# magenta/ddsp

Hardware: AMD Instinct MI355X
Metric: Msamples/s (Harmonic+FilteredNoise, 16kHz, 100 harmonics) (higher is better)
Workload: dtype f32 (Harmonic wavetables and the FilteredNoise FIR/IR products: 22-bit operands - fp16 hi/lo pairs on the MFMA matrix cores - with fp32 accumulation; everything else plain fp32, the frame phase prefix fp64)

## Files before the change

### ddsp_amd/csrc/filtered_noise_mfma.hip

```cpp
#include <hip/hip_runtime.h>
#include <hip/hip_ext.h>
#include <stdint.h>
#include <cstdlib>
#include <type_traits>
#include "../../include/ddsp_amd.h"
#include "common.h"
#include "split_f16.h"
#include "noise_ir65.h"
#include "profile.h"
#include "filtered_noise_mfma.h"
#include "launch.h"

namespace ddsp {

constexpr int kMfWaves = 8;
constexpr int kMfPW = kMfWaves / 2;
constexpr int kMfRows = 8 * kMfPW;
constexpr int kMfFrames = kMfRows - 2;
constexpr int kMfTile = kMfFrames * 64;
constexpr int kMfTapRowBytes = 17 * 16;
constexpr int kMfTapPlane = kMfRows * kMfTapRowBytes;
constexpr int kMfXStride = 80;
constexpr int kMfXElems = 16 + kMfRows * kMfXStride + 16;
constexpr int kMfXPairs = kMfXElems / 2 + 1;
constexpr int kMfXPlane = kMfWaves == 16 ? 10336 : 5216;
static_assert(kMfXPlane >= kMfXPairs * 4 && kMfXPlane % 16 == 0 && (2 * kMfXPlane / 4) % 32 == 16, "noise plane layout");
constexpr int kMfXOGen = kMfXPlane + 96;
static_assert(kMfXOGen % 16 == 0 && (kMfXOGen / 4) % 32 == 16 && kMfWaves == 8, "noise plane layout, generated noise");
template <bool GEN> struct MfX {
  static constexpr int O = GEN ? kMfXOGen : 2 * kMfXPlane;
  static constexpr int BYTES = GEN ? kMfXOGen + kMfXPlane : 4 * kMfXPlane;
};
struct MfHandoff {
  uint4 frag[kMfPW / 2][4][64];
  float last[kMfRows];
  float tap32[kMfRows];
};

struct MfArgs {
  int N, F, start, scale, fs;
  float inv_fs;
  float bias;
  uint32_t k0, k1;
  uint64_t batch_offset;
  int tiles_per_row, n_tiles;
  FastDiv whole_per_row, fs_div;
  int n_whole;
  const float* x_absmax;
  int bits23;
};

static __constant__ Ir65Frags kIr65Frags = make_ir65_frags();

__device__ __forceinline__ void mf_put4(unsigned char* hrow, int t0, float v0, float v1, float v2, float v3) {
  _Float16 h0, l0, h1, l1, h2, l2, h3, l3;
  split(v0, h0, l0); split(v1, h1, l1); split(v2, h2, l2); split(v3, h3, l3);
  unsigned char* q = hrow + t0 * 2;
  *reinterpret_cast<uint2*>(q) = make_uint2(pack(h0, h1), pack(h2, h3));
  *reinterpret_cast<uint2*>(q + kMfTapPlane) = make_uint2(pack(l0, l1), pack(l2, l3));
}
__device__ __forceinline__ void mf_put4_down(unsigned char* hrow, int t1, bool first, float v0, float v1, float v2, float v3) {
  _Float16 h0, l0, h1, l1, h2, l2, h3, l3;
  split(v0, h0, l0); split(v1, h1, l1); split(v2, h2, l2); split(v3, h3, l3);
  unsigned char* q = hrow + (t1 - 3) * 2;
  *reinterpret_cast<uint16_t*>(q) = __builtin_bit_cast(uint16_t, h3);
  *reinterpret_cast<uint16_t*>(q + kMfTapPlane) = __builtin_bit_cast(uint16_t, l3);
  *reinterpret_cast<uint32_t*>(q + 2) = pack(h2, h1);
  *reinterpret_cast<uint32_t*>(q + kMfTapPlane + 2) = pack(l2, l1);
  if (first) {
    *reinterpret_cast<uint16_t*>(q + 6) = __builtin_bit_cast(uint16_t, h0);
    *reinterpret_cast<uint16_t*>(q + kMfTapPlane + 6) = __builtin_bit_cast(uint16_t, l0);
  }
}

template <bool LO>
__device__ __forceinline__ void mf_put_quad(float4 v, int qd, unsigned char* s_xe, unsigned char* s_xo) {
  _Float16 h0, l0, h1, l1, h2, l2, h3, l3;
  split(v.w, h0, l0);
  split(v.z, h1, l1);
  split(v.y, h2, l2);
  split(v.x, h3, l3);
  const int s = qd >> 4, j = 4 * (qd & 15);
  const int u0 = 16 + kMfXStride * s + 60 - j;
  *reinterpret_cast<uint2*>(s_xe + u0 * 2) = make_uint2(pack(h0, h1), pack(h2, h3));
  if (LO) *reinterpret_cast<uint2*>(s_xe + kMfXPlane + u0 * 2) = make_uint2(pack(l0, l1), pack(l2, l3));
  unsigned char* po = s_xo + (u0 + 1) * 2;
  *reinterpret_cast<uint16_t*>(po) = __builtin_bit_cast(uint16_t, h0);
  *reinterpret_cast<uint32_t*>(po + 2) = pack(h1, h2);
  *reinterpret_cast<uint16_t*>(po + 6) = __builtin_bit_cast(uint16_t, h3);
  if (LO) {
    *reinterpret_cast<uint16_t*>(po + kMfXPlane) = __builtin_bit_cast(uint16_t, l0);
    *reinterpret_cast<uint32_t*>(po + kMfXPlane + 2) = pack(l1, l2);
    *reinterpret_cast<uint16_t*>(po + kMfXPlane + 6) = __builtin_bit_cast(uint16_t, l3);
  }
}

template <bool GEN_NOISE, int NLANES>
__device__ __forceinline__ void mf_noise_tile(int ltid, int b, int z0, const float* __restrict__ x, unsigned char* s_xe,
                                              unsigned char* s_xo, const MfArgs& p) {
  int x_exp = 0;
  if constexpr (!GEN_NOISE) {
    if (p.x_absmax) x_exp = pow2_exponent(p.x_absmax[b]);
  }
  if constexpr (GEN_NOISE) {
    static_assert((8 * kMfRows) % NLANES == 0, "octets per lane");
#pragma unroll
    for (int h = 0; h < 8 * kMfRows / NLANES; ++h) {
      const int oc = ltid + NLANES * h;
      const int i = z0 - 128 + 8 * oc;
      float4 v0 = make_float4(0.f, 0.f, 0.f, 0.f), v1 = v0;
      if (i >= 0 && i < p.N) {
        const U4 r = noise_philox(U4{(uint32_t)(i >> 3), (uint32_t)(p.batch_offset + b), 0u, 0u}, p.k0, p.k1);
        v0 = noise_quad(r, 0);
        v1 = noise_quad(r, 1);
        if (i + 7 >= p.N) {
          if (i + 1 >= p.N) v0.y = 0.f;
          if (i + 2 >= p.N) v0.z = 0.f;
          if (i + 3 >= p.N) v0.w = 0.f;
          if (i + 4 >= p.N) v1.x = 0.f;
          if (i + 5 >= p.N) v1.y = 0.f;
          if (i + 6 >= p.N) v1.z = 0.f;
          v1.w = 0.f;
        }
      }
      mf_put_quad<false>(v0, 2 * oc, s_xe, s_xo);
      mf_put_quad<false>(v1, 2 * oc + 1, s_xe, s_xo);
    }
  } else {
    static_assert((16 * kMfRows) % NLANES == 0, "quads per lane");
#pragma unroll
    for (int h = 0; h < 16 * kMfRows / NLANES; ++h) {
      const int qd = ltid + NLANES * h;
      const int i = z0 - 128 + 4 * qd;
      float4 v = make_float4(0.f, 0.f, 0.f, 0.f);
      if (i >= 0 && i < p.N) {
        if (x == nullptr) {
          v = noise_quad_at((uint32_t)i, p.batch_offset + b, p.k0, p.k1, true);
          if (i + 1 >= p.N) v.y = 0.f;
          if (i + 2 >= p.N) v.z = 0.f;
          if (i + 3 >= p.N) v.w = 0.f;
        } else {
          const float* src = x + (size_t)b * p.N + i;
          if (i + 3 < p.N && ((p.N & 3) == 0)) {
            v = *reinterpret_cast<const float4*>(src);
          } else {
            v.x = src[0];
            if (i + 1 < p.N) v.y = src[1];
            if (i + 2 < p.N) v.z = src[2];
            if (i + 3 < p.N) v.w = src[3];
          }
          if (x_exp) { v.x = ldexpf(v.x, -x_exp); v.y = ldexpf(v.y, -x_exp); v.z = ldexpf(v.z, -x_exp); v.w = ldexpf(v.w, -x_exp); }
        }
      }
      mf_put_quad<true>(v, qd, s_xe, s_xo);
    }
  }
}

template <bool GEN_NOISE, bool FS64>
__global__ __launch_bounds__(64 * kMfWaves, 4) void noise_mfma65_kernel(
    const float* __restrict__ mag , const float* __restrict__ x ,
    float* __restrict__ ctl_out , float* __restrict__ out , MfArgs p) {
  __shared__ __attribute__((aligned(16))) unsigned char s_taps_all[2][2 * kMfTapPlane];
  constexpr int kXO = MfX<GEN_NOISE>::O;
  __shared__ __attribute__((aligned(16))) unsigned char s_x_all[2][MfX<GEN_NOISE>::BYTES];
  __shared__ __attribute__((aligned(16))) std::conditional_t<GEN_NOISE, MfHandoff, uint4> s_hand[2];
  __shared__ __attribute__((aligned(16))) float s_carry[2][kMfPW - 1][128];
  const int tid = threadIdx.x, lane = tid & 63;
  const int wave = __builtin_amdgcn_readfirstlane(tid >> 6);
  const int mi = lane & 15, mg = lane >> 4;
  const int n_my = (p.n_tiles - (int)blockIdx.x + (int)gridDim.x - 1) / (int)gridDim.x;
#define DDSP_MF_TILE(T, b_, z0_, ffirst_, rel0_)                                                        \
  const bool last_ = (T) >= p.n_whole;                                                                  \
  uint32_t tx_;                                                                                         \
  const int bq_ = (int)fastdiv((uint32_t)(T), p.whole_per_row, tx_);                                    \
  const int b_ = last_ ? (T) - p.n_whole : bq_;                                                         \
  const int z0_ = (last_ ? p.tiles_per_row - 1 : (int)tx_) * kMfTile;                                   \
  uint32_t fr_;                                                                                         \
  const int fq_ = (int)fastdiv((uint32_t)(z0_ >= 128 ? z0_ - 128 : 128 - z0_ + p.fs - 1), p.fs_div, fr_); \
  const int ffirst_ = (z0_ >= 128) ? fq_ : -fq_;                                                        \
  const int rel0_ = (z0_ - 128) - ffirst_ * p.fs

  if (wave < kMfPW) {
    constexpr bool HANDOFF = GEN_NOISE;
    const float kLog10 = 2.302585092994046f;
    const bool designer = wave < kMfPW / 2;
    const int rg = wave & (kMfPW / 2 - 1);
    if (designer)
      *reinterpret_cast<uint4*>(s_taps_all[lane >> 5] + (lane & 1) * kMfTapPlane + (16 * rg + ((lane >> 1) & 15)) * kMfTapRowBytes + 256) = make_uint4(0u, 0u, 0u, 0u);
    for (int i = tid; i < 2 * (kMfRows + 1) * 16; i += 64 * kMfPW) {
      unsigned char* const s_xe = s_x_all[i >= (kMfRows + 1) * 16 ? 1 : 0];
      unsigned char* const s_xo = s_xe + kXO;
      const int ii = i >= (kMfRows + 1) * 16 ? i - (kMfRows + 1) * 16 : i;
      const int e = 80 * (ii >> 4) + (ii & 15);
      *reinterpret_cast<uint16_t*>(s_xe + e * 2) = 0;
      *reinterpret_cast<uint16_t*>(s_xo + (e + 1) * 2) = 0;
      if (!GEN_NOISE) {
        *reinterpret_cast<uint16_t*>(s_xe + kMfXPlane + e * 2) = 0;
        *reinterpret_cast<uint16_t*>(s_xo + kMfXPlane + (e + 1) * 2) = 0;
      }
    }
    const int rrow = 16 * rg + mi;
    auto group_unused = [&](int rel0, int z0, int f_first) -> bool {
      if (FS64) return false;
      uint32_t r_;
      const int last_tap_row = (int)fastdiv((uint32_t)(rel0 + 64 * (kMfRows - 1)), p.fs_div, r_);
      const int own_hi = (int)fastdiv((uint32_t)(z0 + kMfTile - 128), p.fs_div, r_) + 2;
      return 16 * rg > last_tap_row && 16 * rg >= own_hi - f_first;
    };
    PackedF4 rq[4];
    float r_last;
    auto fetch_rows = [&](int tick_of_tile) {
      const int T = (int)blockIdx.x + min(max(tick_of_tile, 0), n_my - 1) * (int)gridDim.x;
      DDSP_MF_TILE(T, b, z0, f_first, rel0);
      if (group_unused(rel0, z0, f_first)) return;
      const int rfr = f_first + rrow;
      const float* __restrict__ src = mag + ((size_t)b * p.F + ((rfr >= 0 && rfr < p.F) ? rfr : 0)) * 65;
#pragma unroll
      for (int c4 = 0; c4 < 4; ++c4) rq[c4] = *reinterpret_cast<const PackedF4*>(src + 16 * mg + 4 * c4);
      r_last = src[64];
    };
    auto scale_rows = [&](int T, f16x8& be_hi, f16x8& be_lo, f16x8& bo_hi, f16x8& bo_lo, float& m_last, float& t32) -> bool {
      DDSP_MF_TILE(T, b, z0, f_first, rel0);
      const int own_lo = (z0 == 0) ? 0 : f_first + 2;
      uint32_t own_r;
      const int own_hi = (int)fastdiv((uint32_t)(z0 + kMfTile - 128), p.fs_div, own_r) + 2;
      const int rfr = f_first + rrow;
      const bool rvalid = rfr >= 0 && rfr < p.F;
      if (f_first + 16 * rg > p.F + 1 || group_unused(rel0, z0, f_first)) return false;
      float y[16];
#pragma unroll
      for (int c4 = 0; c4 < 4; ++c4) { y[4 * c4] = rq[c4].x; y[4 * c4 + 1] = rq[c4].y; y[4 * c4 + 2] = rq[c4].z; y[4 * c4 + 3] = rq[c4].w; }
      m_last = r_last;
      if (p.scale & 1) {
#pragma unroll
        for (int c = 0; c < 16; ++c) y[c] = exp_sigmoid_fast(y[c] + p.bias, kLog10, 2.0f, 1e-7f);
        m_last = exp_sigmoid_fast(m_last + p.bias, kLog10, 2.0f, 1e-7f);
      }
      if (!rvalid) {
#pragma unroll
        for (int c = 0; c < 16; ++c) y[c] = 0.0f;
        m_last = 0.0f;
      }
      if (ctl_out && rvalid && rfr >= own_lo && rfr < own_hi) {
        float* __restrict__ dst = ctl_out + ((size_t)b * p.F + rfr) * 65;
#pragma unroll
        for (int c4 = 0; c4 < 4; ++c4)
          *reinterpret_cast<PackedF4*>(dst + 16 * mg + 4 * c4) = PackedF4{y[4 * c4], y[4 * c4 + 1], y[4 * c4 + 2], y[4 * c4 + 3]};
        if (mg == 0) dst[64] = m_last;
      }
      float ve[8], vo[8];
#pragma unroll
      for (int e = 0; e < 8; ++e) { ve[e] = y[2 * e]; vo[e] = y[2 * e + 1]; }
      split8(ve, be_hi, be_lo);
      split8(vo, bo_hi, bo_lo);
      const float* __restrict__ c32 = kIr65.c + 32 * kIrRowStride + 8 * mg;
      float part = (mg == 0) ? m_last * kIr65.c[32 * kIrRowStride + 32] : 0.0f;
#pragma unroll
      for (int e = 0; e < 8; ++e) part = fmaf(c32[e], ve[e], part);
      part += __shfl_xor(part, 16);
      part += __shfl_xor(part, 32);
      t32 = kIr65.win[32] * part;
      return true;
    };
    auto make_noise = [&](int tick) {
      if (tick >= 0 && tick + 1 < n_my) {
        const int T = (int)blockIdx.x + (tick + 1) * (int)gridDim.x;
        DDSP_MF_TILE(T, b, z0, f_first, rel0);
        (void)rel0; (void)f_first;
        unsigned char* const s_xe = s_x_all[(tick + 1) & 1];
        if constexpr (HANDOFF) mf_noise_tile<GEN_NOISE, 64 * kMfPW>(tid, b, z0, x, s_xe, s_xe + kXO, p);
        else mf_noise_tile<GEN_NOISE, 32 * kMfPW>(tid - 32 * kMfPW, b, z0, x, s_xe, s_xe + kXO, p);
      }
    };
    if (!designer) {
      if constexpr (HANDOFF) fetch_rows(1);
#pragma unroll 1
      for (int tick = -1; tick < n_my; ++tick) {
        if constexpr (HANDOFF) {
          if (tick + 2 < n_my) {
            const int T = (int)blockIdx.x + (tick + 2) * (int)gridDim.x;
            MfHandoff& h = s_hand[(tick + 2) & 1];
            f16x8 be_hi, be_lo, bo_hi, bo_lo;
            float m_last, t32;
            if (scale_rows(T, be_hi, be_lo, bo_hi, bo_lo, m_last, t32)) {
              h.frag[rg][0][lane] = __builtin_bit_cast(uint4, be_hi);
              h.frag[rg][1][lane] = __builtin_bit_cast(uint4, be_lo);
              h.frag[rg][2][lane] = __builtin_bit_cast(uint4, bo_hi);
              h.frag[rg][3][lane] = __builtin_bit_cast(uint4, bo_lo);
              if (mg == 0) { h.last[rrow] = m_last; h.tap32[rrow] = t32; }
            }
          }
          fetch_rows(tick + 3);
        }
        make_noise(tick);
        __syncthreads();
      }
    } else {
      f16x8 afr[2][2][2];
#pragma unroll
      for (int mt = 0; mt < 2; ++mt)
#pragma unroll
        for (int par = 0; par < 2; ++par)
#pragma unroll
          for (int hl = 0; hl < 2; ++hl) {
            const uint4 v = *reinterpret_cast<const uint4*>(kIr65Frags.v[mt][par][hl][lane]);
            afr[mt][par][hl] = frag(v.x, v.y, v.z, v.w);
          }
      auto design_rows = [&](unsigned char* s_taps, const f16x8& be_hi, const f16x8& be_lo, const f16x8& bo_hi,
                             const f16x8& bo_lo, float m_last, float t32) {
          unsigned char* __restrict__ hrow = s_taps + rrow * kMfTapRowBytes;
          const f32x4 zero = {0.f, 0.f, 0.f, 0.f};
#pragma unroll
          for (int mt = 0; mt < 2; ++mt) {
            f32x4 ea = __builtin_amdgcn_mfma_f32_16x16x32_f16(afr[mt][0][0], be_hi, zero, 0, 0, 0);
            f32x4 oa = __builtin_amdgcn_mfma_f32_16x16x32_f16(afr[mt][1][0], bo_hi, zero, 0, 0, 0);
            f32x4 ex = __builtin_amdgcn_mfma_f32_16x16x32_f16(afr[mt][0][0], be_lo, zero, 0, 0, 0);
            f32x4 ox = __builtin_amdgcn_mfma_f32_16x16x32_f16(afr[mt][1][0], bo_lo, zero, 0, 0, 0);
            ex = __builtin_amdgcn_mfma_f32_16x16x32_f16(afr[mt][0][1], be_hi, ex, 0, 0, 0);
            ox = __builtin_amdgcn_mfma_f32_16x16x32_f16(afr[mt][1][1], bo_hi, ox, 0, 0, 0);
            const f32x4 ev = combine(ea, ex), ov = combine(oa, ox);
            const int n0 = 16 * mt + 4 * mg;
            float g0[4], g1[4];
#pragma unroll
            for (int r = 0; r < 4; ++r) {
              const int n = n0 + r;
              const float e = fmaf(m_last, kIr65.c[n * kIrRowStride + 32], ev[r]);
              const float o = ov[r];
              g0[r] = kIr65.win[n] * (e + o);
              g1[r] = (n >= 1) ? kIr65.win[64 - n] * (e - o) : 0.0f;
            }
            mf_put4(hrow, 64 + n0, g0[0], g0[1], g0[2], g0[3]);
            mf_put4(hrow, n0, g1[0], g1[1], g1[2], g1[3]);
            mf_put4_down(hrow, 64 - n0, true, g0[0], g0[1], g0[2], g0[3]);
            mf_put4_down(hrow, 128 - n0, n0 != 0, g1[0], g1[1], g1[2], g1[3]);
          }
          if (mg == 0) {
            _Float16 h, l;
            split(t32, h, l);
            const uint16_t hb = __builtin_bit_cast(uint16_t, h), lb = __builtin_bit_cast(uint16_t, l);
            *reinterpret_cast<uint16_t*>(hrow + 96 * 2) = hb;
            *reinterpret_cast<uint16_t*>(hrow + kMfTapPlane + 96 * 2) = lb;
            *reinterpret_cast<uint16_t*>(hrow + 32 * 2) = hb;
            *reinterpret_cast<uint16_t*>(hrow + kMfTapPlane + 32 * 2) = lb;
          }
      };
      fetch_rows(0);
      auto designer_tick = [&](int tick, auto scale_here_tag) {
        constexpr bool SCALE_HERE = decltype(scale_here_tag)::value;
        if (tick + 1 < n_my) {
          const int T = (int)blockIdx.x + (tick + 1) * (int)gridDim.x;
          unsigned char* const s_taps = s_taps_all[(tick + 1) & 1];
          if constexpr (SCALE_HERE) {
            f16x8 be_hi, be_lo, bo_hi, bo_lo;
            float m_last = 0.0f, t32 = 0.0f;
            if (scale_rows(T, be_hi, be_lo, bo_hi, bo_lo, m_last, t32)) design_rows(s_taps, be_hi, be_lo, bo_hi, bo_lo, m_last, t32);
          } else if constexpr (HANDOFF) {
            DDSP_MF_TILE(T, b, z0, f_first, rel0);
            (void)b;
            if (f_first + 16 * rg <= p.F + 1 && !group_unused(rel0, z0, f_first)) {
              const MfHandoff& h = s_hand[(tick + 1) & 1];
              design_rows(s_taps, __builtin_bit_cast(f16x8, h.frag[rg][0][lane]), __builtin_bit_cast(f16x8, h.frag[rg][1][lane]),
                          __builtin_bit_cast(f16x8, h.frag[rg][2][lane]), __builtin_bit_cast(f16x8, h.frag[rg][3][lane]),
                          h.last[rrow], h.tap32[rrow]);
            }
          }
        }
        if (!HANDOFF) fetch_rows(tick + 2);
        if constexpr (HANDOFF) make_noise(tick);
        __syncthreads();
      };
      designer_tick(-1, std::true_type{});
#pragma unroll 1
      for (int tick = 0; tick < n_my; ++tick) designer_tick(tick, std::integral_constant<bool, !HANDOFF>{});
    }
  } else {
    const int cw = wave - kMfPW;
    const int p_first = 4 * cw;
    f32x4 kept = {0.f, 0.f, 0.f, 0.f};
    float* kept_ot = nullptr;
    long kept_n = 0;
    int kept_exp = 0;
    const int xsel = ((mi & 1) ? 0 : kXO) + 2 * kMfXStride * 2 * p_first;
    const int second = mg >> 1;
    const int u4 = 79 + kMfXStride * second - 16 * 4 - mi + 8 * (mg & 1);
    const int a_base0 = xsel + ((u4 + 1) >> 1) * 4;
    const int q0 = mi - 4 * second;
    const int b_off = (q0 >= 0 && q0 <= 7) ? (2 * q0 + (mg & 1)) * 16 : 256;
    const int b_ptr0 = (2 * p_first + second) * kMfTapRowBytes + b_off;
    const int lane_off = 16 * mi + 4 * mg;
    auto flush_kept = [&](int parity) {
      if (cw >= 1 && kept_ot != nullptr && mi < 8) {
        const float4 cr = *reinterpret_cast<const float4*>(&s_carry[parity][cw - 1][lane_off]);
        float v[4] = {kept[0] + cr.x, kept[1] + cr.y, kept[2] + cr.z, kept[3] + cr.w};
        if constexpr (!GEN_NOISE) {
#pragma unroll
          for (int r = 0; r < 4; ++r) v[r] = ldexpf(v[r], kept_exp);
        }
#pragma unroll
        for (int r = 0; r < 4; ++r)
          if (kept_n + lane_off + r >= 0 && kept_n + lane_off + r < p.N) kept_ot[lane_off + r] = v[r];
      }
    };
#pragma unroll 1
    for (int tick = -1; tick < n_my; ++tick) {
      if (tick >= 1) flush_kept((tick - 1) & 1);
      if (tick < 0) {
        const int T = (int)blockIdx.x;
        DDSP_MF_TILE(T, b, z0, f_first, rel0);
        (void)f_first; (void)rel0;
        mf_noise_tile<GEN_NOISE, 64 * kMfPW>(tid - 64 * kMfPW, b, z0, x, s_x_all[0], s_x_all[0] + kXO, p);
      }
      bool active = false;
      if (tick >= 0) {
        const int T = (int)blockIdx.x + tick * (int)gridDim.x;
        DDSP_MF_TILE(T, b, z0, f_first, rel0);
        (void)f_first;
        active = (long)z0 - 128 + 128L * p_first - p.start < (long)p.N;
      }
      if (active) {
        const int T = (int)blockIdx.x + tick * (int)gridDim.x;
        DDSP_MF_TILE(T, b, z0, f_first, rel0);
        (void)f_first;
        const unsigned char* const s_taps = s_taps_all[tick & 1];
        const unsigned char* const s_x = s_x_all[tick & 1];
        float* __restrict__ o = out + (size_t)b * p.N;
        const long n_tile = (long)z0 - 128 + 128L * p_first - p.start;
        const bool interior = n_tile + 128 >= 0 && n_tile + 128 * 4 <= (long)p.N && (((p.start | p.N) & 1) == 0);
        float* __restrict__ ot = o + n_tile;
        int o_exp = 0;
        if constexpr (!GEN_NOISE) {
          if (p.x_absmax) o_exp = pow2_exponent(p.x_absmax[b]);
        }
        f32x4 carry = {0.f, 0.f, 0.f, 0.f};
        int a_hi[2], a_lo[2], b_ptr = b_ptr0;
        DDSP_KEEP_IN_VGPR(b_ptr);
        __builtin_assume((b_ptr & 15) == 0);
#pragma unroll
        for (int k = 0; k < 2; ++k) {
          a_hi[k] = a_base0 + 640 * k; a_lo[k] = a_base0 + 640 * k + kMfXPlane;
          DDSP_KEEP_IN_VGPR(a_hi[k]);
          DDSP_KEEP_IN_VGPR(a_lo[k]);
          __builtin_assume((a_hi[k] & 3) == 0);
          __builtin_assume((a_lo[k] & 3) == 0);
        }
        f16x8 fah[3], fal[3], fbh_in[2], fbl_in[2], fbh, fbl;
        auto load_step = [&](int j, int slot) {
          const int it = j / 5, c = j - 5 * it;
          const PackedU4 qh = *reinterpret_cast<const PackedU4*>(s_x + a_hi[it >> 1] + 32 * (4 - c) + 2 * kMfXStride * 2 * (it & 1));
          fah[slot] = frag(qh.x, qh.y, qh.z, qh.w);
          if constexpr (!GEN_NOISE) {
            const PackedU4 ql = *reinterpret_cast<const PackedU4*>(s_x + a_lo[it >> 1] + 32 * (4 - c) + 2 * kMfXStride * 2 * (it & 1));
            fal[slot] = frag(ql.x, ql.y, ql.z, ql.w);
          }
          if (c == 0) {
            const unsigned char* tr;
            if (FS64) {
              tr = s_taps + b_ptr + 2 * kMfTapRowBytes * it;
            } else {
              const int P = p_first + it;
              const int row = (int)(((float)(rel0 + 128 * P + 64 * second) + 0.5f) * p.inv_fs);
              tr = s_taps + row * kMfTapRowBytes + b_off;
            }
            fbh_in[it & 1] = *reinterpret_cast<const f16x8*>(tr);
            fbl_in[it & 1] = *reinterpret_cast<const f16x8*>(tr + kMfTapPlane);
          }
        };
        auto column_up = [](f16x8 v) {
          typedef int i32x4 __attribute__((ext_vector_type(4)));
          const i32x4 w = __builtin_bit_cast(i32x4, v);
          i32x4 o;
#pragma unroll
          for (int k = 0; k < 4; ++k) {
            const int t = w[k];
            o[k] = __builtin_amdgcn_update_dpp(0, t, 0x111, 0xF, 0xF, true);
          }
          return __builtin_bit_cast(f16x8, o);
        };
        load_step(0, 0);
        load_step(1, 1);
        load_step(2, 2);
        __builtin_amdgcn_sched_barrier(0);
        f32x4 acc = {0.f, 0.f, 0.f, 0.f}, acc_hl = {0.f, 0.f, 0.f, 0.f}, acc_lh = {0.f, 0.f, 0.f, 0.f};
        auto pipeline = [&](auto interior_tag) {
          constexpr bool kInterior = decltype(interior_tag)::value;
#pragma unroll
          for (int j = 0; j < 20; ++j) {
            const int it = j / 5, c = j - 5 * it, slot = j % 3;
            if (c == 0) { fbh = fbh_in[it & 1]; fbl = fbl_in[it & 1]; }
            acc = __builtin_amdgcn_mfma_f32_16x16x32_f16(fah[slot], fbh, acc, 0, 0, 0);
            acc_hl = __builtin_amdgcn_mfma_f32_16x16x32_f16(fah[slot], fbl, acc_hl, 0, 0, 0);
            if constexpr (!GEN_NOISE) acc_lh = __builtin_amdgcn_mfma_f32_16x16x32_f16(fal[slot], fbh, acc_lh, 0, 0, 0);
            __builtin_amdgcn_sched_barrier(0);
            if (j + 3 < 20) load_step(j + 3, slot);
            if (c < 4) { fbh = column_up(fbh); fbl = column_up(fbl); }
            __builtin_amdgcn_sched_barrier(0);
            if (c == 4) {
              const f32x4 comb = combine(acc + carry, acc_hl + acc_lh);
              acc = (f32x4){0.f, 0.f, 0.f, 0.f};
              acc_hl = (f32x4){0.f, 0.f, 0.f, 0.f};
              acc_lh = (f32x4){0.f, 0.f, 0.f, 0.f};
              if (it == 0) {
                kept = comb;
              } else if (mi < 8) {
                const int idx = lane_off + 128 * it;
                f32x4 st4 = comb;
                if constexpr (!GEN_NOISE) {
#pragma unroll
                  for (int r = 0; r < 4; ++r) { const float v = comb[r]; st4[r] = ldexpf(v, o_exp); }
                }
                if (kInterior) {
                  *reinterpret_cast<float2*>(ot + idx) = make_float2(st4[0], st4[1]);
                  *reinterpret_cast<float2*>(ot + idx + 2) = make_float2(st4[2], st4[3]);
                } else {
#pragma unroll
                  for (int r = 0; r < 4; ++r) {
                    const float v = st4[r];
                    if (n_tile + idx + r >= 0 && n_tile + idx + r < p.N) ot[idx + r] = v;
                  }
                }
              }
#pragma unroll
              for (int r = 0; r < 4; ++r) {
                const float v = comb[r];
                carry[r] = __builtin_bit_cast(float, __builtin_amdgcn_update_dpp(0, __builtin_bit_cast(int, v), 0x108, 0xF, 0xF, true));
              }
              if (it == 3 && cw < kMfPW - 1 && mi >= 8)
                *reinterpret_cast<float4*>(&s_carry[tick & 1][cw][lane_off - 128]) = make_float4(comb[0], comb[1], comb[2], comb[3]);
            }
          }
        };
        if (interior) pipeline(std::true_type{});
        else pipeline(std::false_type{});
        kept_ot = ot;
        kept_n = n_tile;
        kept_exp = o_exp;
      } else {
        kept_ot = nullptr;
      }
      __syncthreads();
    }
    flush_kept((n_my - 1) & 1);
  }
#undef DDSP_MF_TILE
}

bool noise_mfma65_ok(int F, int M, int N, int padding, const void* noise, int scale) {
  const int frame_size = (N + F - 1) / F;
  return scale != 0 && M == 65 && padding == 0 && frame_size >= 64 && (frame_size % 64) == 0 && frame_size <= 4096 &&
         (N + frame_size - 1) / frame_size == F && (noise == nullptr || (((uintptr_t)noise) & 15) == 0);
}

__global__ __launch_bounds__(1024) void row_absmax_kernel(const float* __restrict__ x, int N, float* __restrict__ out) {
  __shared__ float s_m[16];
  const float* row = x + (size_t)blockIdx.x * N;
  float m = 0.0f;
  for (int i = threadIdx.x; i < N; i += 1024) m = fmaxf(m, fabsf(row[i]));
  m = wave_max_nonneg_dpp(m);
  if ((threadIdx.x & 63) == 0) s_m[threadIdx.x >> 6] = m;
  __syncthreads();
  if (threadIdx.x == 0) {
    float r = 0.0f;
    for (int w = 0; w < 16; ++w) r = fmaxf(r, s_m[w]);
    out[blockIdx.x] = r;
  }
}

int launch_noise_mfma65(const float* magnitudes, const float* noise, float* audio, float* ctl_magnitudes, int B, int F,
                        int N, int start, float initial_bias, int scale, uint64_t seed, uint64_t batch_offset,
                        int bits23, float* row_scratch , hipStream_t st) {
  MfArgs q;
  q.x_absmax = nullptr; q.bits23 = bits23;
  if (noise) {
    if (!row_scratch) return DDSP_ERR_WORKSPACE;
    hipLaunchKernelGGL(row_absmax_kernel, dim3((unsigned)B), dim3(1024), 0, st, noise, N, row_scratch);
    q.x_absmax = row_scratch;
  }
  const bool lo_planes = noise != nullptr || bits23 != 0;
  q.N = N; q.F = F; q.start = start; q.bias = initial_bias; q.scale = scale;
  q.fs = (N + F - 1) / F; q.inv_fs = 1.0f / (float)q.fs;
  q.k0 = (uint32_t)seed; q.k1 = (uint32_t)(seed >> 32); q.batch_offset = batch_offset;
  q.tiles_per_row = (N + start + kMfTile - 1) / kMfTile;
  q.n_tiles = B * q.tiles_per_row;
  q.whole_per_row = make_fastdiv((uint32_t)(q.tiles_per_row > 1 ? q.tiles_per_row - 1 : 1));
  q.fs_div = make_fastdiv((uint32_t)q.fs);
  q.n_whole = B * (q.tiles_per_row - 1);
  static const int n_cu = [] {
    int dev = 0, v = 0;
    if (hipGetDevice(&dev) != hipSuccess ||
        hipDeviceGetAttribute(&v, hipDeviceAttributeMultiprocessorCount, dev) != hipSuccess || v <= 0)
      v = 256;
    return v;
  }();
  const int slots = n_cu * (kMfWaves == 16 ? 1 : 2);
  const dim3 grid((unsigned)(q.n_tiles < slots ? q.n_tiles : slots));
  hipEvent_t ev0, ev1;
  profile_kernel_events(kNoiseMfma, &ev0, &ev1);
#define DDSP_LAUNCH_MF(GEN, FS64)                                                                                      \
  hipExtLaunchKernelGGL((noise_mfma65_kernel<GEN, FS64>), grid, dim3(64 * kMfWaves), 0, st, ev0, ev1, 0, magnitudes, noise, \
                        ctl_magnitudes, audio, q)
  if (q.fs == 64) { if (lo_planes) DDSP_LAUNCH_MF(false, true); else DDSP_LAUNCH_MF(true, true); }
  else { if (lo_planes) DDSP_LAUNCH_MF(false, false); else DDSP_LAUNCH_MF(true, false); }
#undef DDSP_LAUNCH_MF
  return check_launch();
}

}
```

Measured before the change: 114,600.

## Schedule noise tiles as contiguous per-block runs with carry handoff instead of overlap

Replaces the fixed overlapping tile decomposition (each tile recomputed two frames of halo) with contiguous runs of 128-sample pairs per block, split evenly into tiles. The overlap-add carry is passed between consecutive tiles through shared memory, so halo recomputation is avoided and the work per block is balanced. A rounding-order bitmask reproduces the previous summation order at tile seams. This adds per-tile index math and a cross-tile dependency, and rows with few pairs may underfill tiles.

After: 103,900. -9.3%, worse.

```diff
diff --git a/ddsp_amd/csrc/filtered_noise_mfma.hip b/ddsp_amd/csrc/filtered_noise_mfma.hip
--- a/ddsp_amd/csrc/filtered_noise_mfma.hip
+++ b/ddsp_amd/csrc/filtered_noise_mfma.hip
@@ -16,8 +16,9 @@
 constexpr int kMfWaves = 8;
 constexpr int kMfPW = kMfWaves / 2;
 constexpr int kMfRows = 8 * kMfPW;
-constexpr int kMfFrames = kMfRows - 2;
-constexpr int kMfTile = kMfFrames * 64;
+constexpr int kMfPairs = kMfRows / 2;
+constexpr int kMfRoundGrid = 15;
+constexpr uint32_t kMfRoundLate = 0x888u | (0x888u << kMfRoundGrid);
 constexpr int kMfTapRowBytes = 17 * 16;
 constexpr int kMfTapPlane = kMfRows * kMfTapRowBytes;
 constexpr int kMfXStride = 80;
@@ -43,14 +44,43 @@
   float bias;
   uint32_t k0, k1;
   uint64_t batch_offset;
-  int tiles_per_row, n_tiles;
-  FastDiv whole_per_row, fs_div;
-  int n_whole;
+  FastDiv fs_div;
+  int n_runs, run_q, run_rem, tiles_per_run;
+  FastDiv runs_per_row, tiles_per_run_div;
+  int tile_q[3], tile_rem[3];
   const float* x_absmax;
   int bits23;
 };
 
 static __constant__ Ir65Frags kIr65Frags = make_ir65_frags();
+
+struct MfTileAt {
+  int b;
+  int p0;
+  int np;
+  int f_first;
+  int rel0;
+  bool hist;
+  bool carry_in;
+};
+__device__ __forceinline__ MfTileAt mf_tile_at(const MfArgs& p, int k) {
+  MfTileAt t;
+  uint32_t ti, r;
+  const int ri = (int)fastdiv((uint32_t)k, p.tiles_per_run_div, ti);
+  t.b = (int)fastdiv((uint32_t)((int)blockIdx.x + ri * (int)gridDim.x), p.runs_per_row, r);
+  const int hist_run = r > 0 ? 1 : 0;
+  const int cls = ((int)r < p.run_rem ? 1 : 0) + hist_run;
+  const int tq = cls == 0 ? p.tile_q[0] : cls == 1 ? p.tile_q[1] : p.tile_q[2];
+  const int trem = cls == 0 ? p.tile_rem[0] : cls == 1 ? p.tile_rem[1] : p.tile_rem[2];
+  t.p0 = (int)r * p.run_q + min((int)r, p.run_rem) - hist_run + (int)ti * tq + min((int)ti, trem);
+  t.np = tq + ((int)ti < trem ? 1 : 0);
+  t.hist = hist_run && ti == 0;
+  t.carry_in = ti > 0;
+  uint32_t rel;
+  t.f_first = (int)fastdiv((uint32_t)(128 * t.p0), p.fs_div, rel);
+  t.rel0 = (int)rel;
+  return t;
+}
 
 __device__ __forceinline__ void mf_put4(unsigned char* hrow, int t0, float v0, float v1, float v2, float v3) {
   _Float16 h0, l0, h1, l1, h2, l2, h3, l3;
@@ -96,7 +126,7 @@
 }
 
 template <bool GEN_NOISE, int NLANES>
-__device__ __forceinline__ void mf_noise_tile(int ltid, int b, int z0, const float* __restrict__ x, unsigned char* s_xe,
+__device__ __forceinline__ void mf_noise_tile(int ltid, int b, int zs, const float* __restrict__ x, unsigned char* s_xe,
                                               unsigned char* s_xo, const MfArgs& p) {
   int x_exp = 0;
   if constexpr (!GEN_NOISE) {
@@ -107,9 +137,9 @@
 #pragma unroll
     for (int h = 0; h < 8 * kMfRows / NLANES; ++h) {
       const int oc = ltid + NLANES * h;
-      const int i = z0 - 128 + 8 * oc;
+      const int i = zs + 8 * oc;
       float4 v0 = make_float4(0.f, 0.f, 0.f, 0.f), v1 = v0;
-      if (i >= 0 && i < p.N) {
+      if (i < p.N) {
         const U4 r = noise_philox(U4{(uint32_t)(i >> 3), (uint32_t)(p.batch_offset + b), 0u, 0u}, p.k0, p.k1);
         v0 = noise_quad(r, 0);
         v1 = noise_quad(r, 1);
@@ -131,9 +161,9 @@
 #pragma unroll
     for (int h = 0; h < 16 * kMfRows / NLANES; ++h) {
       const int qd = ltid + NLANES * h;
-      const int i = z0 - 128 + 4 * qd;
+      const int i = zs + 4 * qd;
       float4 v = make_float4(0.f, 0.f, 0.f, 0.f);
-      if (i >= 0 && i < p.N) {
+      if (i < p.N) {
         if (x == nullptr) {
           v = noise_quad_at((uint32_t)i, p.batch_offset + b, p.k0, p.k1, true);
           if (i + 1 >= p.N) v.y = 0.f;
@@ -165,21 +195,11 @@
   constexpr int kXO = MfX<GEN_NOISE>::O;
   __shared__ __attribute__((aligned(16))) unsigned char s_x_all[2][MfX<GEN_NOISE>::BYTES];
   __shared__ __attribute__((aligned(16))) std::conditional_t<GEN_NOISE, MfHandoff, uint4> s_hand[2];
-  __shared__ __attribute__((aligned(16))) float s_carry[2][kMfPW - 1][128];
+  __shared__ __attribute__((aligned(16))) float s_carry[2][kMfPW][128];
   const int tid = threadIdx.x, lane = tid & 63;
   const int wave = __builtin_amdgcn_readfirstlane(tid >> 6);
   const int mi = lane & 15, mg = lane >> 4;
-  const int n_my = (p.n_tiles - (int)blockIdx.x + (int)gridDim.x - 1) / (int)gridDim.x;
-#define DDSP_MF_TILE(T, b_, z0_, ffirst_, rel0_)                                                        \
-  const bool last_ = (T) >= p.n_whole;                                                                  \
-  uint32_t tx_;                                                                                         \
-  const int bq_ = (int)fastdiv((uint32_t)(T), p.whole_per_row, tx_);                                    \
-  const int b_ = last_ ? (T) - p.n_whole : bq_;                                                         \
-  const int z0_ = (last_ ? p.tiles_per_row - 1 : (int)tx_) * kMfTile;                                   \
-  uint32_t fr_;                                                                                         \
-  const int fq_ = (int)fastdiv((uint32_t)(z0_ >= 128 ? z0_ - 128 : 128 - z0_ + p.fs - 1), p.fs_div, fr_); \
-  const int ffirst_ = (z0_ >= 128) ? fq_ : -fq_;                                                        \
-  const int rel0_ = (z0_ - 128) - ffirst_ * p.fs
+  const int n_my = (p.n_runs - (int)blockIdx.x + (int)gridDim.x - 1) / (int)gridDim.x * p.tiles_per_run;
 
   if (wave < kMfPW) {
     constexpr bool HANDOFF = GEN_NOISE;
@@ -201,33 +221,32 @@
       }
     }
     const int rrow = 16 * rg + mi;
-    auto group_unused = [&](int rel0, int z0, int f_first) -> bool {
-      if (FS64) return false;
+    auto group_unused = [&](const MfTileAt& t) -> bool {
       uint32_t r_;
-      const int last_tap_row = (int)fastdiv((uint32_t)(rel0 + 64 * (kMfRows - 1)), p.fs_div, r_);
-      const int own_hi = (int)fastdiv((uint32_t)(z0 + kMfTile - 128), p.fs_div, r_) + 2;
-      return 16 * rg > last_tap_row && 16 * rg >= own_hi - f_first;
+      const int last_tap_row = (int)fastdiv((uint32_t)(t.rel0 + 128 * t.np - 64), p.fs_div, r_);
+      const int own_hi = (int)fastdiv((uint32_t)(t.rel0 + 128 * t.np), p.fs_div, r_);
+      return 16 * rg > last_tap_row && 16 * rg >= own_hi;
     };
     PackedF4 rq[4];
     float r_last;
     auto fetch_rows = [&](int tick_of_tile) {
-      const int T = (int)blockIdx.x + min(max(tick_of_tile, 0), n_my - 1) * (int)gridDim.x;
-      DDSP_MF_TILE(T, b, z0, f_first, rel0);
-      if (group_unused(rel0, z0, f_first)) return;
-      const int rfr = f_first + rrow;
-      const float* __restrict__ src = mag + ((size_t)b * p.F + ((rfr >= 0 && rfr < p.F) ? rfr : 0)) * 65;
+      const MfTileAt t = mf_tile_at(p, min(max(tick_of_tile, 0), n_my - 1));
+      if (group_unused(t)) return;
+      const int rfr = t.f_first + rrow;
+      const float* __restrict__ src = mag + ((size_t)t.b * p.F + ((rfr >= 0 && rfr < p.F) ? rfr : 0)) * 65;
 #pragma unroll
       for (int c4 = 0; c4 < 4; ++c4) rq[c4] = *reinterpret_cast<const PackedF4*>(src + 16 * mg + 4 * c4);
       r_last = src[64];
     };
-    auto scale_rows = [&](int T, f16x8& be_hi, f16x8& be_lo, f16x8& bo_hi, f16x8& bo_lo, float& m_last, float& t32) -> bool {
-      DDSP_MF_TILE(T, b, z0, f_first, rel0);
-      const int own_lo = (z0 == 0) ? 0 : f_first + 2;
+    auto scale_rows = [&](int k, f16x8& be_hi, f16x8& be_lo, f16x8& bo_hi, f16x8& bo_lo, float& m_last, float& t32) -> bool {
+      const MfTileAt t = mf_tile_at(p, k);
+      const int b = t.b, f_first = t.f_first;
       uint32_t own_r;
-      const int own_hi = (int)fastdiv((uint32_t)(z0 + kMfTile - 128), p.fs_div, own_r) + 2;
+      const int own_lo = f_first + (int)fastdiv((uint32_t)(t.rel0 + (t.hist ? 128 : 0)), p.fs_div, own_r);
+      const int own_hi = f_first + (int)fastdiv((uint32_t)(t.rel0 + 128 * t.np), p.fs_div, own_r);
       const int rfr = f_first + rrow;
-      const bool rvalid = rfr >= 0 && rfr < p.F;
-      if (f_first + 16 * rg > p.F + 1 || group_unused(rel0, z0, f_first)) return false;
+      const bool rvalid = rfr < p.F;
+      if (f_first + 16 * rg > p.F + 1 || group_unused(t)) return false;
       float y[16];
 #pragma unroll
       for (int c4 = 0; c4 < 4; ++c4) { y[4 * c4] = rq[c4].x; y[4 * c4 + 1] = rq[c4].y; y[4 * c4 + 2] = rq[c4].z; y[4 * c4 + 3] = rq[c4].w; }
@@ -265,12 +284,10 @@
     };
     auto make_noise = [&](int tick) {
       if (tick >= 0 && tick + 1 < n_my) {
-        const int T = (int)blockIdx.x + (tick + 1) * (int)gridDim.x;
-        DDSP_MF_TILE(T, b, z0, f_first, rel0);
-        (void)rel0; (void)f_first;
+        const MfTileAt t = mf_tile_at(p, tick + 1);
         unsigned char* const s_xe = s_x_all[(tick + 1) & 1];
-        if constexpr (HANDOFF) mf_noise_tile<GEN_NOISE, 64 * kMfPW>(tid, b, z0, x, s_xe, s_xe + kXO, p);
-        else mf_noise_tile<GEN_NOISE, 32 * kMfPW>(tid - 32 * kMfPW, b, z0, x, s_xe, s_xe + kXO, p);
+        if constexpr (HANDOFF) mf_noise_tile<GEN_NOISE, 64 * kMfPW>(tid, t.b, 128 * t.p0, x, s_xe, s_xe + kXO, p);
+        else mf_noise_tile<GEN_NOISE, 32 * kMfPW>(tid - 32 * kMfPW, t.b, 128 * t.p0, x, s_xe, s_xe + kXO, p);
       }
     };
     if (!designer) {
@@ -279,11 +296,10 @@
       for (int tick = -1; tick < n_my; ++tick) {
         if constexpr (HANDOFF) {
           if (tick + 2 < n_my) {
-            const int T = (int)blockIdx.x + (tick + 2) * (int)gridDim.x;
             MfHandoff& h = s_hand[(tick + 2) & 1];
             f16x8 be_hi, be_lo, bo_hi, bo_lo;
             float m_last, t32;
-            if (scale_rows(T, be_hi, be_lo, bo_hi, bo_lo, m_last, t32)) {
+            if (scale_rows(tick + 2, be_hi, be_lo, bo_hi, bo_lo, m_last, t32)) {
               h.frag[rg][0][lane] = __builtin_bit_cast(uint4, be_hi);
               h.frag[rg][1][lane] = __builtin_bit_cast(uint4, be_lo);
               h.frag[rg][2][lane] = __builtin_bit_cast(uint4, bo_hi);
@@ -349,16 +365,14 @@
       auto designer_tick = [&](int tick, auto scale_here_tag) {
         constexpr bool SCALE_HERE = decltype(scale_here_tag)::value;
         if (tick + 1 < n_my) {
-          const int T = (int)blockIdx.x + (tick + 1) * (int)gridDim.x;
           unsigned char* const s_taps = s_taps_all[(tick + 1) & 1];
           if constexpr (SCALE_HERE) {
             f16x8 be_hi, be_lo, bo_hi, bo_lo;
             float m_last = 0.0f, t32 = 0.0f;
-            if (scale_rows(T, be_hi, be_lo, bo_hi, bo_lo, m_last, t32)) design_rows(s_taps, be_hi, be_lo, bo_hi, bo_lo, m_last, t32);
+            if (scale_rows(tick + 1, be_hi, be_lo, bo_hi, bo_lo, m_last, t32)) design_rows(s_taps, be_hi, be_lo, bo_hi, bo_lo, m_last, t32);
           } else if constexpr (HANDOFF) {
-            DDSP_MF_TILE(T, b, z0, f_first, rel0);
-            (void)b;
-            if (f_first + 16 * rg <= p.F + 1 && !group_unused(rel0, z0, f_first)) {
+            const MfTileAt t = mf_tile_at(p, tick + 1);
+            if (t.f_first + 16 * rg <= p.F + 1 && !group_unused(t)) {
               const MfHandoff& h = s_hand[(tick + 1) & 1];
               design_rows(s_taps, __builtin_bit_cast(f16x8, h.frag[rg][0][lane]), __builtin_bit_cast(f16x8, h.frag[rg][1][lane]),
                           __builtin_bit_cast(f16x8, h.frag[rg][2][lane]), __builtin_bit_cast(f16x8, h.frag[rg][3][lane]),
@@ -378,6 +392,7 @@
     const int cw = wave - kMfPW;
     const int p_first = 4 * cw;
     f32x4 kept = {0.f, 0.f, 0.f, 0.f};
+    float kept_late = 0.0f;
     float* kept_ot = nullptr;
     long kept_n = 0;
     int kept_exp = 0;
@@ -390,9 +405,22 @@
     const int b_ptr0 = (2 * p_first + second) * kMfTapRowBytes + b_off;
     const int lane_off = 16 * mi + 4 * mg;
     auto flush_kept = [&](int parity) {
-      if (cw >= 1 && kept_ot != nullptr && mi < 8) {
+      if (cw < 1 || kept_ot == nullptr) return;
+      float cross[4];
+#pragma unroll
+      for (int r = 0; r < 4; ++r) {
+        const float kv = kept[r];
+        cross[r] = __builtin_bit_cast(float, __builtin_amdgcn_update_dpp(0, __builtin_bit_cast(int, kv), 0x108, 0xF, 0xF, true));
+      }
+      if (mi < 8) {
         const float4 cr = *reinterpret_cast<const float4*>(&s_carry[parity][cw - 1][lane_off]);
-        float v[4] = {kept[0] + cr.x, kept[1] + cr.y, kept[2] + cr.z, kept[3] + cr.w};
+        const float crv[4] = {cr.x, cr.y, cr.z, cr.w};
+        float v[4];
+#pragma unroll
+        for (int r = 0; r < 4; ++r) {
+          const float kv = kept[r];
+          v[r] = combine(kv + crv[r] * (1.0f - kept_late), cross[r]) + crv[r] * kept_late;
+        }
         if constexpr (!GEN_NOISE) {
 #pragma unroll
           for (int r = 0; r < 4; ++r) v[r] = ldexpf(v[r], kept_exp);
@@ -406,33 +434,30 @@
     for (int tick = -1; tick < n_my; ++tick) {
       if (tick >= 1) flush_kept((tick - 1) & 1);
       if (tick < 0) {
-        const int T = (int)blockIdx.x;
-        DDSP_MF_TILE(T, b, z0, f_first, rel0);
-        (void)f_first; (void)rel0;
-        mf_noise_tile<GEN_NOISE, 64 * kMfPW>(tid - 64 * kMfPW, b, z0, x, s_x_all[0], s_x_all[0] + kXO, p);
-      }
-      bool active = false;
-      if (tick >= 0) {
-        const int T = (int)blockIdx.x + tick * (int)gridDim.x;
-        DDSP_MF_TILE(T, b, z0, f_first, rel0);
-        (void)f_first;
-        active = (long)z0 - 128 + 128L * p_first - p.start < (long)p.N;
-      }
+        const MfTileAt t0 = mf_tile_at(p, 0);
+        mf_noise_tile<GEN_NOISE, 64 * kMfPW>(tid - 64 * kMfPW, t0.b, 128 * t0.p0, x, s_x_all[0], s_x_all[0] + kXO, p);
+      }
+      const MfTileAt t = mf_tile_at(p, max(tick, 0));
+      const bool active = tick >= 0 && p_first < t.np && 128L * (t.p0 + p_first) - p.start < (long)p.N;
       if (active) {
-        const int T = (int)blockIdx.x + tick * (int)gridDim.x;
-        DDSP_MF_TILE(T, b, z0, f_first, rel0);
-        (void)f_first;
+        const int b = t.b, rel0 = t.rel0;
+        const int n_pairs = t.np - p_first;
+        const bool st_first = cw == 0 && !t.hist;
+        const uint32_t late = kMfRoundLate >> ((uint32_t)(t.p0 + p_first) % (uint32_t)kMfRoundGrid);
         const unsigned char* const s_taps = s_taps_all[tick & 1];
         const unsigned char* const s_x = s_x_all[tick & 1];
         float* __restrict__ o = out + (size_t)b * p.N;
-        const long n_tile = (long)z0 - 128 + 128L * p_first - p.start;
-        const bool interior = n_tile + 128 >= 0 && n_tile + 128 * 4 <= (long)p.N && (((p.start | p.N) & 1) == 0);
+        const long n_tile = 128L * (t.p0 + p_first) - p.start;
+        const bool interior = n_pairs >= 4 && n_tile + (st_first ? 0 : 128) >= 0 && n_tile + 128 * 4 <= (long)p.N &&
+                              (((p.start | p.N) & 1) == 0);
         float* __restrict__ ot = o + n_tile;
         int o_exp = 0;
         if constexpr (!GEN_NOISE) {
           if (p.x_absmax) o_exp = pow2_exponent(p.x_absmax[b]);
         }
         f32x4 carry = {0.f, 0.f, 0.f, 0.f};
+        const bool take_in = cw == 0 && t.carry_in && mi < 8;
+        const float* const s_in = &s_carry[(tick - 1) & 1][kMfPW - 1][lane_off & 127];
         int a_hi[2], a_lo[2], b_ptr = b_ptr0;
         DDSP_KEEP_IN_VGPR(b_ptr);
         __builtin_assume((b_ptr & 15) == 0);
@@ -495,14 +520,33 @@
             if (j + 3 < 20) load_step(j + 3, slot);
             if (c < 4) { fbh = column_up(fbh); fbl = column_up(fbl); }
             __builtin_amdgcn_sched_barrier(0);
+            if (j == 4) {
+              const float4 c_in = *reinterpret_cast<const float4*>(s_in);
+              carry = take_in ? (f32x4){c_in.x, c_in.y, c_in.z, c_in.w} : (f32x4){0.f, 0.f, 0.f, 0.f};
+            }
             if (c == 4) {
-              const f32x4 comb = combine(acc + carry, acc_hl + acc_lh);
+              const f32x4 cross = acc_hl + acc_lh;
+              const bool is_late = (late >> it) & 1u;
+              f32x4 comb;
+              if (is_late) {
+                __asm__ volatile("");
+                comb = combine(acc, cross) + carry;
+              } else {
+                comb = combine(acc + carry, cross);
+              }
+              if (it == 0) {
+#pragma unroll
+                for (int r = 0; r < 4; ++r) {
+                  const float av = acc[r], xv = cross[r];
+                  kept[r] = __builtin_bit_cast(float, __builtin_amdgcn_update_dpp(__builtin_bit_cast(int, av), __builtin_bit_cast(int, xv),
+                                                                                  0x118, 0xF, 0xC, false));
+                }
+                kept_late = is_late ? 1.0f : 0.0f;
+              }
               acc = (f32x4){0.f, 0.f, 0.f, 0.f};
               acc_hl = (f32x4){0.f, 0.f, 0.f, 0.f};
               acc_lh = (f32x4){0.f, 0.f, 0.f, 0.f};
-              if (it == 0) {
-                kept = comb;
-              } else if (mi < 8) {
+              if ((it > 0 || st_first) && mi < 8) {
                 const int idx = lane_off + 128 * it;
                 f32x4 st4 = comb;
                 if constexpr (!GEN_NOISE) {
@@ -516,7 +560,7 @@
 #pragma unroll
                   for (int r = 0; r < 4; ++r) {
                     const float v = st4[r];
-                    if (n_tile + idx + r >= 0 && n_tile + idx + r < p.N) ot[idx + r] = v;
+                    if (it < n_pairs && n_tile + idx + r >= 0 && n_tile + idx + r < p.N) ot[idx + r] = v;
                   }
                 }
               }
@@ -525,8 +569,10 @@
                 const float v = comb[r];
                 carry[r] = __builtin_bit_cast(float, __builtin_amdgcn_update_dpp(0, __builtin_bit_cast(int, v), 0x108, 0xF, 0xF, true));
               }
-              if (it == 3 && cw < kMfPW - 1 && mi >= 8)
-                *reinterpret_cast<float4*>(&s_carry[tick & 1][cw][lane_off - 128]) = make_float4(comb[0], comb[1], comb[2], comb[3]);
+              const bool tile_last = (!kInterior || it == 3) && it == n_pairs - 1;
+              if (((it == 3 && cw < kMfPW - 1) || tile_last) && mi >= 8)
+                *reinterpret_cast<float4*>(&s_carry[tick & 1][tile_last ? kMfPW - 1 : cw][lane_off - 128]) =
+                    make_float4(comb[0], comb[1], comb[2], comb[3]);
             }
           }
         };
@@ -542,7 +588,6 @@
     }
     flush_kept((n_my - 1) & 1);
   }
-#undef DDSP_MF_TILE
 }
 
 bool noise_mfma65_ok(int F, int M, int N, int padding, const void* noise, int scale) {
@@ -580,11 +625,7 @@
   q.N = N; q.F = F; q.start = start; q.bias = initial_bias; q.scale = scale;
   q.fs = (N + F - 1) / F; q.inv_fs = 1.0f / (float)q.fs;
   q.k0 = (uint32_t)seed; q.k1 = (uint32_t)(seed >> 32); q.batch_offset = batch_offset;
-  q.tiles_per_row = (N + start + kMfTile - 1) / kMfTile;
-  q.n_tiles = B * q.tiles_per_row;
-  q.whole_per_row = make_fastdiv((uint32_t)(q.tiles_per_row > 1 ? q.tiles_per_row - 1 : 1));
   q.fs_div = make_fastdiv((uint32_t)q.fs);
-  q.n_whole = B * (q.tiles_per_row - 1);
   static const int n_cu = [] {
     int dev = 0, v = 0;
     if (hipGetDevice(&dev) != hipSuccess ||
@@ -592,8 +633,22 @@
       v = 256;
     return v;
   }();
-  const int slots = n_cu * (kMfWaves == 16 ? 1 : 2);
-  const dim3 grid((unsigned)(q.n_tiles < slots ? q.n_tiles : slots));
+  const int slots = n_cu * 2;
+  const int row_pairs = (N + start + 127) / 128;
+  int runs_per_row = slots / B > 1 ? slots / B : 1;
+  if (runs_per_row > row_pairs / kMfPairs) runs_per_row = row_pairs / kMfPairs > 1 ? row_pairs / kMfPairs : 1;
+  q.n_runs = B * runs_per_row;
+  q.runs_per_row = make_fastdiv((uint32_t)runs_per_row);
+  q.run_q = row_pairs / runs_per_row;
+  q.run_rem = row_pairs % runs_per_row;
+  const int longest = q.run_q + (runs_per_row > 1 ? (q.run_rem > 1 ? 2 : 1) : 0);
+  q.tiles_per_run = (longest + kMfPairs - 1) / kMfPairs;
+  q.tiles_per_run_div = make_fastdiv((uint32_t)q.tiles_per_run);
+  for (int i = 0; i < 3; ++i) {
+    q.tile_q[i] = (q.run_q + i) / q.tiles_per_run;
+    q.tile_rem[i] = (q.run_q + i) % q.tiles_per_run;
+  }
+  const dim3 grid((unsigned)(q.n_runs < slots ? q.n_runs : slots));
   hipEvent_t ev0, ev1;
   profile_kernel_events(kNoiseMfma, &ev0, &ev1);
 #define DDSP_LAUNCH_MF(GEN, FS64)                                                                                      \
```
